# priyasundaresan/panda-lang-manip

Hardware: AMD Instinct MI355X
Metric: env steps/sec (batched) PandaPush-v3 at 1/2/4/8 MI355X vs PyBullet CPU (higher is better)
Workload: dtype f32; 1 GPU; PandaPush-v3 x65536/gpu; env_id=PandaPush-v3, task=push, control=ee, reward=sparse, batch_per_gpu=65536, global_batch=65536, substeps=20, parallelism=batch shard x1, lanes_per_env=1

## Files before the change

panda-lang-manip_amd/csrc/ps_scene.h:

```cpp
#pragma once

#include "ps_common.h"

namespace ps {

constexpr int SHAPE_BOX = PS_SHAPE_BOX;
constexpr int SHAPE_CYL = PS_SHAPE_CYLINDER;

struct Scene {
    V3 base;
    V3 half;
    float mass, mass2, fric;
    float table_cx, table_hx, table_hy;
    int has_table, has_plane;
};

struct Motors {
    float target[9], kp[9], kd[9], vel[9], imp[9];
};

struct Body {
    V3 pos;
    Q4 quat;
    V3 vel, omg;
// ... 77 lines not shown
PS_D V3 support_point(const Scene &sc) {
    if constexpr (SHAPE == SHAPE_CYL) {
        constexpr int order[PM_CYL_RIM_POINTS] = PM_CYL_RIM_ORDER;
        constexpr int cap = V / PM_CYL_RIM_POINTS;
        constexpr int j = order[V % PM_CYL_RIM_POINTS];
        constexpr float cs[8] = {1.0f, 0.70710678118654752f, 0.0f, -0.70710678118654752f,
                                 -1.0f, -0.70710678118654752f, 0.0f, 0.70710678118654752f};
        constexpr float sn[8] = {0.0f, 0.70710678118654752f, 1.0f, 0.70710678118654752f,
                                 0.0f, -0.70710678118654752f, -1.0f, -0.70710678118654752f};
        return mk(sc.half.x * cs[j], sc.half.x * sn[j], cap ? sc.half.z : -sc.half.z);
    } else {
        return mk((V & 1) ? sc.half.x : -sc.half.x, (V & 2) ? sc.half.y : -sc.half.y,
                  (V & 4) ? sc.half.z : -sc.half.z);
    }
}

template <int SHAPE>
PS_D float object_closest(const Scene &sc, V3 loc, V3 &cl, V3 &nl) {
    const V3 h = sc.half;
    if constexpr (SHAPE == SHAPE_CYL) {
        float r = h.x, hh = h.z;
        float rho = fast_sqrt(loc.x * loc.x + loc.y * loc.y);
        float zc = fminf(fmaxf(loc.z, -hh), hh);
        float irho = fast_rcp(rho);
        float s = rho > r ? r * irho : 1.0f;
        cl = mk(loc.x * s, loc.y * s, zc);
        V3 dif = loc - cl;
        float dn = fast_norm(dif);
        if (dn > 1e-9f) {
            nl = dif * fast_rcp(dn);
            return dn;
        }
        float side = r - rho, cap = hh - fabsf(loc.z);
        if (side < cap) {
            nl = rho > 1e-12f ? mk(loc.x * irho, loc.y * irho, 0.0f) : mk(1.0f, 0.0f, 0.0f);
            cl = mk(nl.x * r, nl.y * r, cl.z);
            return -side;
        }
        nl = mk(0.0f, 0.0f, loc.z >= 0.0f ? 1.0f : -1.0f);
        cl.z = nl.z * hh;
        return -cap;
    } else {
        cl = mk(fminf(fmaxf(loc.x, -h.x), h.x), fminf(fmaxf(loc.y, -h.y), h.y), fminf(fmaxf(loc.z, -h.z), h.z));
        V3 dif = loc - cl;
        float dn = norm(dif);
        if (dn > 1e-9f) {
            nl = dif * (1.0f / dn);
            return dn;
        }
        float bx = h.x - fabsf(loc.x), by = h.y - fabsf(loc.y), bz = h.z - fabsf(loc.z);
        int ax = 0;
        float best = bx;
        if (by < best) { best = by; ax = 1; }
        if (bz < best) { best = bz; ax = 2; }
        float sg;
        if (ax == 0) { sg = loc.x >= 0.0f ? 1.0f : -1.0f; nl = mk(sg, 0, 0); cl.x = sg * h.x; }
        else if (ax == 1) { sg = loc.y >= 0.0f ? 1.0f : -1.0f; nl = mk(0, sg, 0); cl.y = sg * h.y; }
        else { sg = loc.z >= 0.0f ? 1.0f : -1.0f; nl = mk(0, 0, sg); cl.z = sg * h.z; }
        return -best;
    }
}

PS_D void plane_space(V3 n, V3 &p, V3 &q) {
    if (fabsf(n.z) > 0.70710678118654752f) {
        float a = n.y * n.y + n.z * n.z, k = rsqrtf(a);
        p = mk(0.0f, -n.z * k, n.y * k);
        q = mk(a * k, -n.x * p.z, n.x * p.y);
    } else {
        float a = n.x * n.x + n.y * n.y, k = rsqrtf(a);
        p = mk(-n.y * k, n.x * k, 0.0f);
        q = mk(-n.z * p.y, n.z * p.x, a * k);
    }
}

constexpr int NG = PM_MAX_GROUND_CONTACTS;
constexpr int NR = PM_MAX_ROBOT_CONTACTS;
constexpr int NP = PM_MAX_PAIR_CONTACTS;
constexpr int LDS_STASH_OFFSET = NR * 27;
constexpr int LDS_STASH_FLOATS = 40;
constexpr int LDS_CACHE_OFFSET = LDS_STASH_OFFSET + LDS_STASH_FLOATS;
constexpr int LDS_CACHE_FLOATS = 10;
constexpr int LDS_FLOATS = LDS_CACHE_OFFSET + LDS_CACHE_FLOATS;
static_assert(LDS_FLOATS * 4 * 64 * 4 <= 160 * 1024, "four workgroups per CU");
constexpr int LDS_GND_OFFSET = NR * 27;
constexpr int LDS_GND_FLOATS = 6;
constexpr int LDS_FLOATS_STACK = LDS_GND_OFFSET + 2 * NG * LDS_GND_FLOATS;
static_assert(LDS_FLOATS_STACK * 4 * 64 * 4 <= 160 * 1024, "four Stack workgroups per CU");
constexpr int PAIR_FLOATS = 21;
constexpr int GSTASH_ROWS = LDS_STASH_FLOATS + 13 - 9;
constexpr int GSTASH_PAIR_OFFSET = GSTASH_ROWS;
constexpr int GSTASH_ZERO_FLOATS = 32;
constexpr int GRIP_MJ_SLOTS = NR;
constexpr int GSTASH_GRIP_OFFSET = GSTASH_PAIR_OFFSET + NP * PAIR_FLOATS;
constexpr int GRIP_FLOATS = GRIP_MJ_SLOTS * 9;
constexpr int GSTASH_FLOATS = GSTASH_GRIP_OFFSET + GRIP_FLOATS;
template <int NOBJ>
constexpr int lds_floats() {
    return NOBJ == 2 ? LDS_FLOATS_STACK : LDS_FLOATS;
}

struct GroundContact {
    V3 r;
    float rhs[3], lam[3], dinv[3];
    int id;
};

struct PairContact {
    V3 dir[3], rA, rB;
    float rhs[3], lam[3], dinv[3];
    bool a0;
};

struct RobotContact {
    float J[3][9];
    V3 dir[3];
    V3 rn[3];
    float rhs[3], lam[3], dinv[3], mu;
    bool o1;
};

typedef __attribute__((address_space(3))) float lds_float;
struct MJStore {
    lds_float *base;
    int stride;
    lds_float *cwo = nullptr;
    PS_D lds_float &at(int slot, int row, int k) const { return base[((slot * 3 + row) * 9 + k) * stride]; }
    PS_D lds_float &cache(int k) const { return base[(LDS_CACHE_OFFSET + k) * stride]; }
    PS_D lds_float &stash(int k) const { return base[(LDS_STASH_OFFSET + k) * stride]; }
    float *gst = nullptr;
    int64_t gst_stride = 0;
    uint32_t goff = 0;
    __attribute__((address_space(1))) float *gpair = nullptr;
    PS_D float &gstash(int k) const {
        float *row = gst + k * gst_stride;
        asm("" : "+s"(row));
        return *(float *)((char *)row + goff);
    }
    PS_D lds_float &gnd(int c, int k) const { return base[(LDS_GND_OFFSET + c * LDS_GND_FLOATS + k) * stride]; }
    PS_D float &pair(int c, int k) const { return *(float *)&gpair[c * PAIR_FLOATS + k]; }
    __attribute__((address_space(1))) float *ggrip = nullptr;
    PS_D float &grip(int c, int k) const { return *(float *)&ggrip[c * 9 + k]; }
    __attribute__((address_space(1))) float *gzero = nullptr;
    PS_D __attribute__((address_space(1))) float *pair_rows(int c, int n) const {
        return c < n ? gpair + c * PAIR_FLOATS : gzero;
    }
    PS_D __attribute__((address_space(1))) float *grip_rows(int c, int n) const {
        return c < n ? ggrip + c * 9 : gzero;
    }
    PS_D MJStore opaque() const {
        MJStore r = *this;
        asm volatile("" : "+v"(r.base));
        asm volatile("" : "+v"(r.goff));
        asm volatile("" : "+v"(r.gpair));
        asm volatile("" : "+v"(r.ggrip));
        return r;
    }
};

struct VelChange {
    f32x2 p[4];
    float z;
    PS_D float g(int a) const { return a == 8 ? z : p[a >> 1][a & 1]; }
    PS_D void s(int a, float v) {
        if (a == 8) z = v;
        else p[a >> 1][a & 1] = v;
    }
    PS_D f32x2 bc(int a) const {
        if (a == 8) return (f32x2){z, z};
        return (a & 1) ? __builtin_shufflevector(p[a >> 1], p[a >> 1], 1, 1)
                       : __builtin_shufflevector(p[a >> 1], p[a >> 1], 0, 0);
    }
    PS_D void apply(const float m[9], float sc) {
#pragma unroll
        for (int k = 0; k < 4; k++)
            p[k] = __builtin_elementwise_fma((f32x2){m[2 * k], m[2 * k + 1]}, (f32x2){sc, sc}, p[k]);
        z = fmaf(m[8], sc, z);
    }
    PS_D float dot(const float J[9]) const {
        float acc = 0.0f;
#pragma unroll
        for (int a = 0; a < 9; a++) acc = fmaf(J[a], g(a), acc);
        return acc;
    }
};

PS_D V3 pk_fma3(V3 a, float s, V3 c) {
    const f32x2 xy = __builtin_elementwise_fma((f32x2){a.x, a.y}, (f32x2){s, s}, (f32x2){c.x, c.y});
    return mk(xy.x, xy.y, fmaf(a.z, s, c.z));
}

PS_D float jrow_dot(const float J[9], const float v[9]) {
    float s = 0.0f;
#pragma unroll
    for (int d = 0; d < 9; d++) s += J[d] * v[d];
    return s;
}

struct Geo {
    V3 ax[9], org[7], bc[PM_NUM_BOXES], wc;
    M3 hR;
};

}
```

panda-lang-manip_amd/csrc/ps_substep.h:

```cpp
#pragma once

#include "ps_collide.h"
#include "ps_dynamics.h"
#include "ps_solver.h"
#include "ps_solver_group.h"

namespace ps {

#ifdef PS_PROFILE_PHASES
#define PS_COUNT_IT() prof_it++
#else
#define PS_COUNT_IT() do {} while (0)
#endif
#define PS_REGATE()                                                                        \
    do {                                                                                   \
        asm volatile("" : "+s"(gate_lim), "+s"(gate_pair), "+s"(gate_robot));              \
        for (int b_ = 0; b_ < NB; b_++) asm volatile("" : "+s"(gate_ground[b_]));         \
    } while (0)

struct LimitSide {
    float pen, sgn;
    bool on, combined;
    PS_D float split() const { return sgn * (-pen) * (float)PM_SPLIT_LIMIT_ERP; }
};
PS_D LimitSide limit_side(int d, int side, float qd_) {
    const double LO = dof_def(d).lo, HI = dof_def(d).hi;
    const float lo_h = (float)LO, lo_t = (float)(LO - (double)lo_h);
    const float hi_h = (float)HI, hi_t = (float)(HI - (double)hi_h);
    LimitSide s;
    s.pen = side ? (hi_h - qd_) + hi_t : (qd_ - lo_h) - lo_t;
    s.sgn = side ? -1.0f : 1.0f;
    s.on = s.pen <= 0.0f;
    s.combined = s.pen > (float)PM_SPLIT_PENETRATION_THRESHOLD;
    return s;
}

PS_D float split_of(int d, float qd_) {
    float split = 0.0f;
#pragma unroll
    for (int side = 0; side < 2; side++) {
        const LimitSide s = limit_side(d, side, qd_);
        if (s.on && !s.combined) split += s.split();
    }
    return split;
}

template <int NOBJ, int SHAPE, bool STD_MOTORS, int G = 1>
PS_D void substep(const Scene &sc, float q[9], float qd[9], const Motors &mt, Body *bd, const MJStore &lds,
                  const WarmCache<G, NOBJ> &wc PS_PROF_PARAM PS_DUMP_PARAM) {
    static_assert(NOBJ >= 0 && NOBJ <= 2, "objects");
    static_assert(NOBJ < 2 || SHAPE == SHAPE_BOX, "Stack stacks cubes");
    constexpr int NB = NOBJ > 0 ? NOBJ : 1;
    constexpr bool ANISO = SHAPE == SHAPE_CYL;
    const float dt = (float)PM_TIMESTEP;
    float Mi[45], hb[9];
    Geo geo;
    bias_forces(q, qd, hb);
    PS_PHASE(0);
    __builtin_amdgcn_sched_barrier(0);
    {
        Kin k;
        fk(q, k);
        static_for<0, 9>([&](auto D) {
            constexpr int d = decltype(D)::value;
            geo.ax[d] = dof_axis<d>(k);
            if constexpr (d < 7) geo.org[d] = k.f[d].o;
        });
        geo.hR = k.f[8].R;
        static_for<0, PM_NUM_BOXES>([&](auto BB) {
            constexpr int B = decltype(BB)::value;
            constexpr BoxDef b = box_def(B);
            geo.bc[B] = k.f[b.link].o + mul(k.f[b.link].R, mk((float)b.c[0], (float)b.c[1], (float)b.c[2])) + sc.base;
        });
        {
            constexpr SphereDef w = wrist_def();
            geo.wc = k.f[w.link].o + mul(k.f[w.link].R, mk((float)w.c[0], (float)w.c[1], (float)w.c[2])) + sc.base;
        }
        mass_matrix(k, Mi);
    }
#ifdef PS_PROFILE_PHASES
#pragma unroll
    for (int k = 0; k < 45; k++) asm volatile("" ::"v"(Mi[k]));
#endif
    PS_PHASE(1);
    __builtin_amdgcn_sched_barrier(0);
    spd_inverse(Mi);
#ifdef PS_PROFILE_PHASES
#pragma unroll
    for (int k = 0; k < 45; k++) asm volatile("" ::"v"(Mi[k]));
#endif
    PS_PHASE(2);
    __builtin_amdgcn_sched_barrier(0);
    int nr;
    {
        M3 oR[NB];
#pragma unroll
        for (int b = 0; b < NB; b++) oR[b] = NOBJ > 0 ? quat_to_mat(bd[b].quat) : M3{{1, 0, 0, 0, 1, 0, 0, 0, 1}};
        nr = robot_candidates<NOBJ, SHAPE, G>(sc, geo, bd, oR, lds PS_PROF_ARG);
    }
    PS_PHASE(17);
    __builtin_amdgcn_sched_barrier(0);
    float v1[9];
#pragma unroll
    for (int a = 0; a < 9; a++) {
        float s = 0.0f;
#pragma unroll
        for (int b = 0; b < 9; b++) s -= Mi[sidx(a, b)] * hb[b];
        v1[a] = qd[a] + dt * s;
    }
    V3 cw1[NB], cv1[NB];
    BodyDyn<SHAPE> od[NB];
#pragma unroll
    for (int b = 0; b < NB; b++) {
        cw1[b] = mk(0, 0, 0);
        cv1[b] = mk(0, 0, 0);
    }
#pragma unroll
    for (int b = 0; b < NOBJ; b++) {
        od[b] = body_dyn<SHAPE>(sc, bd[b], b == 0 ? sc.mass : sc.mass2);
        float cl = (float)PM_LINEAR_DAMPING + (float)PM_LINEAR_DAMPING * norm(bd[b].vel);
        float ca = (float)PM_ANGULAR_DAMPING + (float)PM_ANGULAR_DAMPING * norm(bd[b].omg);
        cv1[b] = bd[b].vel + (mk(0, 0, (float)PM_GRAVITY_Z) - bd[b].vel * cl) * dt;
        cw1[b] = bd[b].omg - bd[b].omg * (ca * dt);
        if constexpr (ANISO) {
            V3 I = local_inertia<SHAPE>(sc, b == 0 ? sc.mass : sc.mass2);
            S3 Iw = rotate_diag(od[b].R, I.x, I.y, I.z);
            V3 gyro = od[b].inv_inertia(cross(bd[b].omg, mul(Iw, bd[b].omg)));
            cw1[b] = cw1[b] - gyro * dt;
        }
    }

    float dinvj[9];
    float lim_rhs[9], lim_lam[9];
    unsigned lim_on = 0u, lim_up = 0u;
    float split_dq[9];
    float mot_rhs[9], mot_lam[9];
// ... 104 lines not shown
        float pl[NP];
        V3 ppt[NP];
        const int pn = (int)wc.load(PS_F_WPN);
#pragma unroll
        for (int k = 0; k < NP; k++) {
            pl[k] = wc.load(PS_F_WP + k);
            ppt[k] = mk(wc.load(PS_F_WPPT + 3 * k), wc.load(PS_F_WPPT + 3 * k + 1), wc.load(PS_F_WPPT + 3 * k + 2));
        }
#pragma unroll
        for (int c = 0; c < NP; c++) {
            PairContact &p = pc[c];
            if (c < np) {
                const PairCand &cd = cand[c];
                int A = cd.a0 ? 0 : 1;
                V3 dirs[3];
                dirs[0] = cd.n;
                plane_space(cd.n, dirs[1], dirs[2]);
                V3 rA = cd.pA - (A == 0 ? bd[0].pos : bd[1].pos), rB = cd.pB - (A == 0 ? bd[1].pos : bd[0].pos);
                p.a0 = cd.a0;
                p.rA = A == 0 ? rA : rB;
                p.rB = A == 0 ? rB : rA;
#pragma unroll
                for (int j = 0; j < 3; j++) {
                    V3 dj = dirs[j];
                    p.dir[j] = dj;
                    const V3 rnA = cross(rA, dj), rnB = cross(rB, dj);
                    float iIA = A == 0 ? od[0].iI : od[1].iI, iIB = A == 0 ? od[1].iI : od[0].iI;
                    float imA = A == 0 ? od[0].inv_m : od[1].inv_m, imB = A == 0 ? od[1].inv_m : od[0].inv_m;
                    float den = dot(rnA, rnA) * iIA + dot(rnB, rnB) * iIB + dot(dj, dj) * (imA + imB);
                    p.dinv[j] = safe_inv(den);
                    V3 wA = A == 0 ? cw1[0] : cw1[1], vA = A == 0 ? cv1[0] : cv1[1];
                    V3 wB = A == 0 ? cw1[1] : cw1[0], vB = A == 0 ? cv1[1] : cv1[0];
                    float rel = dot(rnA, wA) + dot(dj, vA) - dot(rnB, wB) - dot(dj, vB);
                    p.lam[j] = 0.0f;
                    p.rhs[j] = j == 0 ? normal_rhs(cd.dist, rel, p.dinv[0]) : -rel * p.dinv[j];
                }
                V3 lp = tmul(od[0].R, cd.pB - bd[0].pos);
                float best = (float)(PM_CONTACT_BREAKING_THRESHOLD * PM_CONTACT_BREAKING_THRESHOLD), l0 = 0.0f;
#pragma unroll
                for (int k = 0; k < NP; k++) {
                    V3 d = ppt[k] - lp;
                    float d2 = dot(d, d);
                    bool hit = k < pn && d2 < best;
                    best = hit ? d2 : best;
                    l0 = hit ? pl[k] : l0;
                }
                p.lam[0] = warm * l0;
                wc.store(PS_F_WPPT + 3 * c, lp.x);
                wc.store(PS_F_WPPT + 3 * c + 1, lp.y);
                wc.store(PS_F_WPPT + 3 * c + 2, lp.z);
            } else {
                p.a0 = true;
                p.rA = p.rB = mk(0, 0, 0);
#pragma unroll
                for (int j = 0; j < 3; j++) {
                    p.dir[j] = mk(0, 0, 0);
                    p.rhs[j] = p.lam[j] = p.dinv[j] = 0.0f;
                }
            }
            if (c < np) {
#pragma unroll
                for (int j = 0; j < 3; j++) {
                    lds.pair(c, 3 * j + 0) = p.dir[j].x; lds.pair(c, 3 * j + 1) = p.dir[j].y; lds.pair(c, 3 * j + 2) = p.dir[j].z;
                    lds.pair(c, 15 + j) = p.rhs[j];
                    lds.pair(c, 18 + j) = p.dinv[j];
                }
                lds.pair(c, 9) = p.rA.x; lds.pair(c, 10) = p.rA.y; lds.pair(c, 11) = p.rA.z;
                lds.pair(c, 12) = p.rB.x; lds.pair(c, 13) = p.rB.y; lds.pair(c, 14) = p.rB.z;
            }
        }
        wc.store(PS_F_WPN, (float)np);
    }
    RobotContact rc[NR];
    {
        PS_PHASE(18);
        float prl[NR];
#pragma unroll
        for (int k = 0; k < NR; k++) prl[k] = wc.load(PS_F_WR + k);
        const unsigned prid = (unsigned)wc.load(PS_F_WRID);
        unsigned nrid = 0u;
#pragma unroll
        for (int sl = 0; sl < NR; sl++) {
            RobotContact &c = rc[sl];
            if (sl < nr) {
                const RobotCand cd = RobotCand::load(lds, sl);
                V3 dirs[3];
                dirs[0] = cd.n;
                plane_space(cd.n, dirs[1], dirs[2]);
                c.mu = cd.mu;
                c.o1 = cd.obj == 1;
                bool on_obj = NOBJ > 0 && cd.obj >= 0;
                V3 p = cd.pA - sc.base;
                V3 opos = NOBJ == 2 && cd.obj == 1 ? bd[NB - 1].pos : bd[0].pos;
                V3 rB = cd.pB - opos;
                V3 ow = NOBJ == 2 && cd.obj == 1 ? cw1[NB - 1] : cw1[0];
                V3 ov = NOBJ == 2 && cd.obj == 1 ? cv1[NB - 1] : cv1[0];
                float oim = NOBJ == 2 && cd.obj == 1 ? od[NB - 1].inv_m : od[0].inv_m;
#pragma unroll
                for (int j = 0; j < 3; j++) {
                    V3 dj = dirs[j];
#pragma unroll
                    for (int D = 0; D < 7; D++) c.J[j][D] = dot(geo.ax[D], cross(p - geo.org[D], dj));
                    c.J[j][7] = cd.link == 9 ? dot(geo.ax[7], dj) : 0.0f;
                    c.J[j][8] = cd.link == 10 ? dot(geo.ax[8], dj) : 0.0f;
                    float den = 0.0f;
#pragma unroll
                    for (int a = 0; a < 9; a++) {
                        float s = 0.0f;
#pragma unroll
                        for (int b = 0; b < 9; b++) s += Mi[sidx(a, b)] * c.J[j][b];
                        lds.at(sl, j, a) = NOBJ == 2 ? c.J[j][a] : s;
                        if constexpr (NOBJ == 2)
                            if (j == 0) lds.grip(sl, a) = s;
                        den += c.J[j][a] * s;
                    }
                    float rel = jrow_dot(c.J[j], v1);
                    c.rn[j] = on_obj ? cross(rB, dj) : mk(0, 0, 0);
                    c.dir[j] = on_obj ? dj : mk(0, 0, 0);
                    if constexpr (NOBJ > 0) {
                        V3 w = ANISO ? od[0].inv_inertia(c.rn[j])
                                     : c.rn[j] * (NOBJ == 2 && cd.obj == 1 ? od[NB - 1].iI : od[0].iI);
                        if (on_obj) {
                            den += dot(c.rn[j], w) + dot(dj, dj) * oim;
                            rel -= dot(c.rn[j], ow) + dot(dj, ov);
                        }
                    }
                    c.dinv[j] = safe_inv(den);
                    c.lam[j] = 0.0f;
                    c.rhs[j] = j == 0 ? normal_rhs(cd.dist, rel, c.dinv[0]) : -rel * c.dinv[j];
                }
                c.lam[0] = warm * cache_lookup(prl, prid, (unsigned)cd.id);
                nrid |= (unsigned)cd.id << (5 * sl);
            } else {
                c.mu = 0.0f;
                c.o1 = false;
#pragma unroll
                for (int j = 0; j < 3; j++) {
#pragma unroll
                    for (int a = 0; a < 9; a++) {
                        c.J[j][a] = 0.0f;
                        lds.at(sl, j, a) = 0.0f;
                    }
                    c.dir[j] = c.rn[j] = mk(0, 0, 0);
                    c.rhs[j] = c.lam[j] = c.dinv[j] = 0.0f;
                }
            }
        }
        wc.store(PS_F_WRID, (float)nrid);
    }
    PS_PHASE(3);
    __builtin_amdgcn_sched_barrier(0);
    auto gk = [](int k) { return NOBJ == 2 && k >= 27 ? k - 9 : k; };
    auto put = [&](int k, float v) {
        if constexpr (NOBJ == 2) lds.gstash(gk(k)) = v;
        else lds.stash(k) = v;
    };
    auto get = [&](const MJStore &S, int k) -> float {
        if constexpr (NOBJ == 2) return S.gstash(gk(k));
        else return S.stash(k);
    };
#pragma unroll
    for (int d = 0; d < 9; d++) {
        put(d, q[d]);
        put(9 + d, v1[d]);
        if constexpr (NOBJ != 2) put(18 + d, split_dq[d]);
    }
    if constexpr (NOBJ > 0) {
        put(27, cw1[0].x); put(28, cw1[0].y); put(29, cw1[0].z);
        put(30, cv1[0].x); put(31, cv1[0].y); put(32, cv1[0].z);
        put(33, bd[0].pos.x); put(34, bd[0].pos.y); put(35, bd[0].pos.z);
        put(36, bd[0].quat.x); put(37, bd[0].quat.y); put(38, bd[0].quat.z); put(39, bd[0].quat.w);
    }
    if constexpr (NOBJ == 2) {
        put(40, cw1[1].x); put(41, cw1[1].y); put(42, cw1[1].z);
        put(43, cv1[1].x); put(44, cv1[1].y); put(45, cv1[1].z);
        put(46, bd[1].pos.x); put(47, bd[1].pos.y); put(48, bd[1].pos.z);
        put(49, bd[1].quat.x); put(50, bd[1].quat.y); put(51, bd[1].quat.z); put(52, bd[1].quat.w);
    }

    float dv[9];
#pragma unroll
    for (int d = 0; d < 9; d++) dv[d] = 0.0f;
    V3 dw[NB], dvl[NB];
#pragma unroll
    for (int b = 0; b < NB; b++) {
        dw[b] = mk(0, 0, 0);
        dvl[b] = mk(0, 0, 0);
    }
    float res;
    MJStore L = lds;

    auto wave_bits = [&](auto pred, int n) {
        unsigned m = 0u;
        for (int k = 0; k < n; k++) m |= __builtin_amdgcn_ballot_w64(pred(k)) ? 1u << k : 0u;
        return (unsigned)__builtin_amdgcn_readfirstlane((int)m);
    };
    unsigned gate_lim = wave_bits([&](int d) { return ((lim_on >> d) & 1u) != 0u; }, 9);
    unsigned gate_ground[NB];
#pragma unroll
    for (int b = 0; b < NB; b++) gate_ground[b] = wave_bits([&](int c) { return c < ng[b]; }, NG);
    unsigned gate_pair = wave_bits([&](int c) { return c < np; }, NP);
    unsigned gate_robot = wave_bits([&](int c) { return c < nr; }, NR);

#ifdef PS_PROFILE_PHASES
    int prof_it = 0;
#endif
    static_assert(PM_SOLVER_ITERATIONS % 2 == 0, "iteration pairs");
    if constexpr (G == 1) {
        VelChange dvv;
#pragma unroll
        for (int k = 0; k < 4; k++) dvv.p[k] = (f32x2){0.0f, 0.0f};
        dvv.z = 0.0f;
        auto mcol_apply = [&](int d, float f) {
            const int a0 = (d + 1) & ~1;
#pragma unroll
            for (int a = 0; a < 9; a++)
                if (a < a0 || a == 8) dvv.s(a, fmaf(Mi[sidx(a, d)], f, dvv.g(a)));
#pragma unroll
            for (int a = a0; a < 8; a += 2)
                dvv.p[a >> 1] = __builtin_elementwise_fma((f32x2){Mi[sidx(a, d)], Mi[sidx(a + 1, d)]}, (f32x2){f, f},
                                                          dvv.p[a >> 1]);
        };
        auto joint_row = [&](int d, float sgn, float rhs, float &lam, float lo, float hi) {
            float dl = rhs - dinvj[d] * (sgn * dvv.g(d));
            float nl = clamp_impulse(lam + dl, lo, hi);
            dl = nl - lam;
            lam = nl;
            mcol_apply(d, sgn * dl);
            res = res_max(res, joint_viol(dl, Mi[sidx(d, d)]));
        };
        auto limit_row = [&](int d) {
            if (PS_GATE(gate_lim & (1u << d), 0)) {
                float sgn = (lim_up >> d) & 1u ? -1.0f : 1.0f;
                float hi = (lim_on >> d) & 1u ? (float)PM_LIMIT_MAX_IMPULSE : 0.0f;
                joint_row(d, sgn, lim_rhs[d], lim_lam[d], 0.0f, hi);
            }
        };
        auto motor_row = [&](int d) {
            float imp = STD_MOTORS ? (float)(joint_force(d) * PM_TIMESTEP) : mt.imp[d];
            joint_row(d, 1.0f, mot_rhs[d], mot_lam[d], -imp, imp);
        };
        auto obj_add = [&](bool o1, V3 ddw, V3 ddv) {
            if constexpr (NOBJ == 2) {
                const float s1 = o1 ? 1.0f : 0.0f, s0 = o1 ? 0.0f : 1.0f;
                dw[0] = fma3(ddw, s0, dw[0]);
                dvl[0] = fma3(ddv, s0, dvl[0]);
                dw[NB - 1] = fma3(ddw, s1, dw[NB - 1]);
                dvl[NB - 1] = fma3(ddv, s1, dvl[NB - 1]);
            } else {
                dw[0] = dw[0] + ddw;
                dvl[0] = dvl[0] + ddv;
            }
        };
        auto obj_dw = [&](bool o1) { return NOBJ == 2 && o1 ? dw[NB - 1] : dw[0]; };
        auto obj_dv = [&](bool o1) { return NOBJ == 2 && o1 ? dvl[NB - 1] : dvl[0]; };
        auto pair_rel = [&](V3 rn0, V3 rn1, V3 d) {
            return dot(rn0, dw[0]) + dot(d, dvl[0]) - dot(rn1, dw[NB - 1]) - dot(d, dvl[NB - 1]);
        };
        auto pair_apply = [&](V3 rn0, V3 rn1, V3 d, float sdl) {
            dw[0] = pk_fma3(rn0, sdl * od[0].iI, dw[0]);
            dvl[0] = pk_fma3(d, sdl * od[0].inv_m, dvl[0]);
            dw[NB - 1] = pk_fma3(rn1, -sdl * od[NB - 1].iI, dw[NB - 1]);
            dvl[NB - 1] = pk_fma3(d, -sdl * od[NB - 1].inv_m, dvl[NB - 1]);
        };

        auto mi_apply = [&](const float g[9]) {
#pragma unroll
            for (int b = 0; b < 9; b++) mcol_apply(b, g[b]);
        };

        {
            MJStore W = lds.opaque();
#pragma unroll
            for (int b = 0; b < NOBJ; b++)
#pragma unroll
                for (int c = 0; c < NG; c++)
                    if (PS_GATE(gate_ground[b] & (1u << c), 1)) {
                        const float l0 = gc[b][c].lam[0];
                        V3 gr = gc[b][c].r;
                        if (NOBJ == 2) {
                            const int at = b * NG + c;
                            gr = mk(W.gnd(at, 0), W.gnd(at, 1), W.gnd(at, 2));
                        }
                        dw[b] = dw[b] + od[b].inv_inertia(mk(gr.y * l0, -gr.x * l0, 0.0f));
                        dvl[b].z = fmaf(l0, od[b].inv_m, dvl[b].z);
                    }
            if constexpr (NOBJ == 2) {
#pragma unroll
                for (int c = 0; c < NP; c++)
                    if (gate_pair & (1u << c)) {
                        const auto *pr = W.pair_rows(c, np);
                        auto pv = [&](int k) { return mk(pr[k], pr[k + 1], pr[k + 2]); };
                        const float sl = pc[c].a0 ? pc[c].lam[0] : -pc[c].lam[0];
                        const V3 d0 = pv(0);
                        pair_apply(cross(pv(9), d0), cross(pv(12), d0), d0, sl);
                    }
            }
#pragma unroll
            for (int c = 0; c < NR; c++)
                if (PS_GATE(gate_robot & (1u << c), c < 2)) {
                    const RobotContact &r = rc[c];
                    const float l0 = r.lam[0];
                    float Jl[9];
#pragma unroll
                    for (int a = 0; a < 9; a++) Jl[a] = NOBJ == 2 ? (float)W.at(c, 0, a) : r.J[0][a];
                    if constexpr (NOBJ == 2) {
                        float g[9];
#pragma unroll
                        for (int a = 0; a < 9; a++) g[a] = Jl[a] * l0;
                        mi_apply(g);
                    } else {
                        float w[9];
#pragma unroll
                        for (int a = 0; a < 9; a++) w[a] = W.at(c, 0, a);
#pragma unroll
                        for (int a = 0; a < 9; a++) dvv.s(a, fmaf(w[a], l0, dvv.g(a)));
                    }
                    if constexpr (NOBJ > 0) {
                        float im = NOBJ == 2 && r.o1 ? od[NB - 1].inv_m : od[0].inv_m;
                        V3 ddw = ANISO ? od[0].inv_inertia(r.rn[0] * -l0)
                                       : r.rn[0] * (-l0 * (NOBJ == 2 && r.o1 ? od[NB - 1].iI : od[0].iI));
                        obj_add(r.o1, ddw, r.dir[0] * (-l0 * im));
                    }
                }
        }

        float gmj[GRIP_MJ_SLOTS][9];
        auto object_normals = [&]() {
            if constexpr (NOBJ == 2) {
                float pf[NP][11];
                if constexpr (NOBJ == 2) {
                    if (gate_pair) {
#pragma unroll
                        for (int c = 0; c < NP; c++) {
                            const auto *pr = L.pair_rows(c, np);
#pragma unroll
                            for (int k = 0; k < 3; k++) {
                                pf[c][k] = pr[k];
                                pf[c][3 + k] = pr[9 + k];
                                pf[c][6 + k] = pr[12 + k];
                            }
                            pf[c][9] = pr[15];
                            pf[c][10] = pr[18];
                        }
                        __builtin_amdgcn_sched_barrier(0);
                    }
                    {
#pragma unroll
                        for (int c = 0; c < GRIP_MJ_SLOTS; c++)
                            if (gate_robot & (1u << c)) {
                                const auto *gr = L.grip_rows(c, nr);
#pragma unroll
                                for (int k = 0; k < 9; k++) gmj[c][k] = gr[k];
                            }
                        __builtin_amdgcn_sched_barrier(0);
                    }
                }
#pragma unroll
                for (int b = 0; b < NOBJ; b++) {
                    const float inv_m = od[b].inv_m;
#pragma unroll
                    for (int c = 0; c < NG; c++) {
                        GroundContact &g = gc[b][c];
                        V3 gr = g.r;
                        float grhs = g.rhs[0], gdinv = g.dinv[0];
                        if (NOBJ == 2) {
                            const int at = b * NG + c;
                            gr = mk(L.gnd(at, 0), L.gnd(at, 1), L.gnd(at, 2));
                            grhs = L.gnd(at, 3);
                            gdinv = c < ng[b] ? cube_ground_dinv(gr, 0, od[b].iI, inv_m) : 0.0f;
                        }
                        V3 rn = mk(gr.y, -gr.x, 0.0f);
                        float dl = grhs - gdinv * (rn.x * dw[b].x + rn.y * dw[b].y + dvl[b].z);
                        float nl = clamp_impulse(g.lam[0] + dl, 0.0f, (float)PM_CONTACT_UPPER);
                        dl = nl - g.lam[0];
                        g.lam[0] = nl;
                        if constexpr (ANISO) {
                            dw[b] = dw[b] + od[b].inv_inertia(mk(rn.x * dl, rn.y * dl, 0.0f));
                        } else {
                            float dI = dl * od[b].iI;
                            dw[b].x = fmaf(rn.x, dI, dw[b].x);
                            dw[b].y = fmaf(rn.y, dI, dw[b].y);
                        }
                        dvl[b].z = fmaf(dl, inv_m, dvl[b].z);
                        res = res_max(res, row_viol(dl, gdinv));
                    }
                }
                if constexpr (NOBJ == 2) {
                    if (gate_pair) {
#pragma unroll
                        for (int c = 0; c < NP; c++)
                            if (gate_pair & (1u << c)) {
                                PairContact &p = pc[c];
                                const float sg = p.a0 ? 1.0f : -1.0f;
                                const V3 d0 = mk(pf[c][0], pf[c][1], pf[c][2]);
                                const V3 rn0 = cross(mk(pf[c][3], pf[c][4], pf[c][5]), d0);
                                const V3 rn1 = cross(mk(pf[c][6], pf[c][7], pf[c][8]), d0);
                                float jv = sg * pair_rel(rn0, rn1, d0);
                                float dl = pf[c][9] - pf[c][10] * jv;
                                float nl = clamp_impulse(p.lam[0] + dl, 0.0f, (float)PM_CONTACT_UPPER);
                                dl = nl - p.lam[0];
                                p.lam[0] = nl;
                                pair_apply(rn0, rn1, d0, sg * dl);
                                res = res_max(res, row_viol(dl, pf[c][10]));
                            }
                    }
                }
            }
        };
        auto contacts = [&]() {
#pragma unroll
            for (int c = 0; c < NR; c++)
                if (PS_GATE(gate_robot & (1u << c), c < 2)) {
                    RobotContact &r = rc[c];
                    float mj[9], Jl[9];
#pragma unroll
                    for (int a = 0; a < 9; a++) Jl[a] = NOBJ == 2 ? (float)L.at(c, 0, a) : r.J[0][a];
                    if constexpr (NOBJ != 2) {
#pragma unroll
                        for (int a = 0; a < 9; a++) mj[a] = L.at(c, 0, a);
                    }
                    __builtin_amdgcn_sched_barrier(0);
                    float jv = dvv.dot(Jl);
                    if (NOBJ > 0) jv -= dot(r.rn[0], obj_dw(r.o1)) + dot(r.dir[0], obj_dv(r.o1));
                    float dl = r.rhs[0] - r.dinv[0] * jv;
                    float nl = clamp_impulse(r.lam[0] + dl, 0.0f, (float)PM_CONTACT_UPPER);
                    dl = nl - r.lam[0];
                    r.lam[0] = nl;
                    if constexpr (NOBJ == 2) {
                        dvv.apply(gmj[c], dl);
                    } else {
                        dvv.apply(mj, dl);
                    }
                    if constexpr (NOBJ == 1) {
                        dw[0] = ANISO ? dw[0] + od[0].inv_inertia_pk(r.rn[0] * -dl) : pk_fma3(r.rn[0], -dl * od[0].iI, dw[0]);
                        dvl[0] = pk_fma3(r.dir[0], -dl * od[0].inv_m, dvl[0]);
                    } else if constexpr (NOBJ == 2) {
                        float im = r.o1 ? od[NB - 1].inv_m : od[0].inv_m;
                        float iI = r.o1 ? od[NB - 1].iI : od[0].iI;
                        obj_add(r.o1, r.rn[0] * (-dl * iI), r.dir[0] * (-dl * im));
                    }
                    res = res_max(res, row_viol(dl, r.dinv[0]));
                }
            float pq[NP][16];
            if constexpr (NOBJ == 2) {
                if (gate_pair) {
#pragma unroll
                    for (int c = 0; c < NP; c++) {
                        const auto *pr = L.pair_rows(c, np);
#pragma unroll
                        for (int k = 0; k < 12; k++) pq[c][k] = pr[3 + k];
                        pq[c][12] = pr[16];
                        pq[c][13] = pr[17];
                        pq[c][14] = pr[19];
                        pq[c][15] = pr[20];
                    }
                    __builtin_amdgcn_sched_barrier(0);
                }
            }

#pragma unroll
            for (int b = 0; b < NOBJ; b++) {
                const float inv_m = od[b].inv_m;
#pragma unroll
                for (int c = 0; c < NG; c++)
                    if (PS_GATE(gate_ground[b] & (1u << c), 1)) {
                        GroundContact &g = gc[b][c];
                        V3 gr = g.r;
                        float grhs1 = g.rhs[1], grhs2 = g.rhs[2], gdinv1 = g.dinv[1], gdinv2 = g.dinv[2];
                        if (NOBJ == 2) {
                            const int at = b * NG + c;
                            gr = mk(L.gnd(at, 0), L.gnd(at, 1), L.gnd(at, 2));
                            grhs1 = L.gnd(at, 4);
                            grhs2 = L.gnd(at, 5);
                            const bool on = c < ng[b];
                            gdinv1 = on ? cube_ground_dinv(gr, 1, od[b].iI, inv_m) : 0.0f;
                            gdinv2 = on ? cube_ground_dinv(gr, 2, od[b].iI, inv_m) : 0.0f;
                        }
                        float dla, dlb;
                        {
#pragma clang fp contract(off)
                            const f32x2 gz = {gr.z, gr.z};
                            const f32x2 t = (f32x2){gr.x, gr.y} * (f32x2){dw[b].z, dw[b].z};
                            const f32x2 u = __builtin_elementwise_fma(gz, (f32x2){dw[b].x, dw[b].y}, -t);
                            const f32x2 w = u + (f32x2){-dvl[b].y, dvl[b].x};
                            const f32x2 lam12 = {g.lam[1], g.lam[2]};
                            const f32x2 s2 = lam12 + __builtin_elementwise_fma(-(f32x2){gdinv1, gdinv2}, w,
                                                                               (f32x2){grhs1, grhs2});
                            const float lim = gmu * g.lam[0];
                            const float m2 = NOBJ == 2 ? fmaf(s2.x, s2.x, s2.y * s2.y) : fmaf(s2.y, s2.y, s2.x * s2.x);
                            const float sc2 = cone_scale(m2, lim);
                            const f32x2 dl2 = __builtin_elementwise_fma(s2, (f32x2){sc2, sc2}, -lam12);
                            const f32x2 nl2 = s2 * (f32x2){sc2, sc2};
                            g.lam[1] = nl2.x;
                            g.lam[2] = nl2.y;
                            dla = dl2.x;
                            dlb = dl2.y;
                            if constexpr (ANISO) {
                                const f32x2 zab = gz * dl2;
                                dw[b] = dw[b] + od[b].inv_inertia_pk_unfused(mk(zab.x, zab.y, fmaf(-gr.x, dla, -gr.y * dlb)));
                            } else {
                                const f32x2 ab = dl2 * (f32x2){od[b].iI, od[b].iI};
                                const f32x2 wxy = __builtin_elementwise_fma(gz, ab, (f32x2){dw[b].x, dw[b].y});
                                dw[b].z = fmaf(-gr.y, ab.y, fmaf(-gr.x, ab.x, dw[b].z));
                                dw[b].x = wxy.x;
                                dw[b].y = wxy.y;
                            }
                            const f32x2 vxy = __builtin_elementwise_fma((f32x2){dlb, -dla}, (f32x2){inv_m, inv_m},
                                                                        (f32x2){dvl[b].x, dvl[b].y});
                            dvl[b].x = vxy.x;
                            dvl[b].y = vxy.y;
                        }
                        res = res_max(res, res_max(row_viol(dla, gdinv1), row_viol(dlb, gdinv2)));
                    }
            }
            if constexpr (NOBJ == 2) {
                const float pmu = sc.fric * sc.fric;
                if (gate_pair) {
#pragma unroll
                    for (int c = 0; c < NP; c++)
                        if (gate_pair & (1u << c)) {
                            PairContact &p = pc[c];
                            auto pv = [&](int k) { return mk(pq[c][k], pq[c][k + 1], pq[c][k + 2]); };
                            const float sg = p.a0 ? 1.0f : -1.0f;
                            const V3 d1 = pv(0), d2 = pv(3), r0 = pv(6), r1 = pv(9);
                            const V3 rn01 = cross(r0, d1), rn02 = cross(r0, d2), rn11 = cross(r1, d1), rn12 = cross(r1, d2);
                            float ja = sg * pair_rel(rn01, rn11, d1);
                            float jb = sg * pair_rel(rn02, rn12, d2);
                            float dla = pq[c][12] - pq[c][14] * ja, dlb = pq[c][13] - pq[c][15] * jb;
                            float sa = p.lam[1] + dla, sb = p.lam[2] + dlb;
                            float lim = pmu * p.lam[0];
                            float m2 = sa * sa + sb * sb;
                            float s = cone_scale(m2, lim);
                            sa *= s;
                            sb *= s;
                            dla = sa - p.lam[1];
                            dlb = sb - p.lam[2];
                            p.lam[1] = sa;
                            p.lam[2] = sb;
                            pair_apply(rn01, rn11, d1, sg * dla);
                            pair_apply(rn02, rn12, d2, sg * dlb);
                            res = res_max(res, res_max(row_viol(dla, pq[c][14]), row_viol(dlb, pq[c][15])));
                        }
                }
            }
#pragma unroll
            for (int c = 0; c < NR; c++)
                if (PS_GATE(gate_robot & (1u << c), c < 2)) {
                    RobotContact &r = rc[c];
                    float mj1[9], mj2[9], J1[9], J2[9];
#pragma unroll
                    for (int a = 0; a < 9; a++) {
                        J1[a] = NOBJ == 2 ? (float)L.at(c, 1, a) : r.J[1][a];
                        J2[a] = NOBJ == 2 ? (float)L.at(c, 2, a) : r.J[2][a];
                    }
                    if constexpr (NOBJ != 2) {
#pragma unroll
                        for (int a = 0; a < 9; a++) {
                            mj1[a] = L.at(c, 1, a);
                            mj2[a] = L.at(c, 2, a);
                        }
                    }
                    __builtin_amdgcn_sched_barrier(0);
                    float ja, jb;
                    if constexpr (NOBJ != 2) {
#pragma clang fp contract(off)
                        f32x2 j2 = {0.0f, 0.0f};
#pragma unroll
                        for (int a = 0; a < 9; a++) j2 = __builtin_elementwise_fma((f32x2){J1[a], J2[a]}, dvv.bc(a), j2);
                        ja = j2.x;
                        jb = j2.y;
                    } else {
                        ja = dvv.dot(J1);
                        jb = dvv.dot(J2);
                    }
                    if (NOBJ > 0) {
                        V3 ow = obj_dw(r.o1), ov = obj_dv(r.o1);
                        ja -= dot(r.rn[1], ow) + dot(r.dir[1], ov);
                        jb -= dot(r.rn[2], ow) + dot(r.dir[2], ov);
                    }
                    float dla, dlb;
                    if constexpr (NOBJ != 2) {
#pragma clang fp contract(off)
                        const f32x2 lam12 = {r.lam[1], r.lam[2]};
                        const f32x2 s2 = lam12 + __builtin_elementwise_fma(-(f32x2){r.dinv[1], r.dinv[2]}, (f32x2){ja, jb},
                                                                           (f32x2){r.rhs[1], r.rhs[2]});
                        const float lim = r.mu * r.lam[0];
                        const float sc2 = cone_scale(fmaf(s2.x, s2.x, s2.y * s2.y), lim);
                        const f32x2 dl2 = __builtin_elementwise_fma(s2, (f32x2){sc2, sc2}, -lam12);
                        const f32x2 nl2 = s2 * (f32x2){sc2, sc2};
                        r.lam[1] = nl2.x;
                        r.lam[2] = nl2.y;
                        dla = dl2.x;
                        dlb = dl2.y;
                    } else {
                        dla = r.rhs[1] - r.dinv[1] * ja;
                        dlb = r.rhs[2] - r.dinv[2] * jb;
                        float sa = r.lam[1] + dla, sb = r.lam[2] + dlb;
                        const float lim = r.mu * r.lam[0];
                        const float m2 = sa * sa + sb * sb;
                        const float s = cone_scale(m2, lim);
                        sa *= s;
                        sb *= s;
                        dla = sa - r.lam[1];
                        dlb = sb - r.lam[2];
                        r.lam[1] = sa;
                        r.lam[2] = sb;
                    }
                    if constexpr (NOBJ == 2) {
                        float g[9];
#pragma unroll
                        for (int a = 0; a < 9; a++) g[a] = fmaf(J2[a], dlb, J1[a] * dla);
                        mi_apply(g);
                    } else {
                        dvv.apply(mj1, dla);
                        dvv.apply(mj2, dlb);
                    }
                    if constexpr (NOBJ == 1) {
                        if constexpr (ANISO) {
                            dw[0] = dw[0] + od[0].inv_inertia_pk(fma3(r.rn[2], -dlb, r.rn[1] * -dla));
                        } else {
                            float aI = -dla * od[0].iI, bI = -dlb * od[0].iI;
                            dw[0] = pk_fma3(r.rn[2], bI, pk_fma3(r.rn[1], aI, dw[0]));
                        }
                        float am = -dla * od[0].inv_m, bm = -dlb * od[0].inv_m;
                        dvl[0] = pk_fma3(r.dir[2], bm, pk_fma3(r.dir[1], am, dvl[0]));
                    } else if constexpr (NOBJ == 2) {
                        float im = r.o1 ? od[NB - 1].inv_m : od[0].inv_m;
                        float iI = r.o1 ? od[NB - 1].iI : od[0].iI;
                        float aI = -dla * iI, bI = -dlb * iI;
                        V3 ddw = mk(fmaf(r.rn[2].x, bI, r.rn[1].x * aI), fmaf(r.rn[2].y, bI, r.rn[1].y * aI),
                                    fmaf(r.rn[2].z, bI, r.rn[1].z * aI));
                        float am = -dla * im, bm = -dlb * im;
                        V3 ddv = mk(fmaf(r.dir[2].x, bm, r.dir[1].x * am), fmaf(r.dir[2].y, bm, r.dir[1].y * am),
                                    fmaf(r.dir[2].z, bm, r.dir[1].z * am));
                        obj_add(r.o1, ddw, ddv);
                    }
                    res = res_max(res, res_max(row_viol(dla, r.dinv[1]), row_viol(dlb, r.dinv[2])));
                }
// ... 25 lines not shown
        for (int it = 0; it < PM_SOLVER_ITERATIONS; it += 2) {
            PS_COUNT_IT();
            L = lds.opaque();
            res = 0.0f;
            PS_REGATE();
            if constexpr (NOBJ == 1) {
#pragma unroll
                for (int k = 0; k < 45; k++) asm volatile("" : "+v"(Mi[k]));
            }
#pragma unroll
            for (int d = 8; d >= 0; d--) motor_row(d);
            ground_normals();
            object_normals();
            if (PS_GATE(gate_lim != 0u, 0)) {
#pragma unroll
                for (int d = 8; d >= 0; d--) limit_row(d);
            }
            contacts();
            if (res <= 0.0f) break;
            PS_COUNT_IT();
            L = lds.opaque();
            res = 0.0f;
            PS_REGATE();
            if (PS_GATE(gate_lim != 0u, 0)) {
#pragma unroll
                for (int d = 0; d < 9; d++) limit_row(d);
            }
#pragma unroll
            for (int d = 0; d < 9; d++) motor_row(d);
            ground_normals();
            object_normals();
            contacts();
            if (res <= 0.0f) break;
        }
#pragma unroll
        for (int a = 0; a < 9; a++) dv[a] = dvv.g(a);
    } else {
        group_pgs<NOBJ, SHAPE, STD_MOTORS, G>(mt, Mi, lds, gate_lim, lim_up, lim_on, gate_ground[0], gate_robot,
                                              dinvj, lim_rhs, lim_lam, mot_rhs, mot_lam, gc[0], rc, od[0], gmu,
                                              dv, dw[0], dvl[0] PS_PROF_COUNT_ARG PS_DUMP_ARG);
    }

#pragma unroll
    for (int b = 0; b < NOBJ; b++)
#pragma unroll
        for (int c = 0; c < NG; c++) wc.store((b == 0 ? PS_F_WG0 : PS_F_WG1) + c, gc[b][c].lam[0]);
    if constexpr (NOBJ == 2) {
#pragma unroll
        for (int c = 0; c < NP; c++) wc.store(PS_F_WP + c, pc[c].lam[0]);
    }
#pragma unroll
    for (int c = 0; c < NR; c++) wc.store(PS_F_WR + c, rc[c].lam[0]);

    PS_PHASE(4);
#ifdef PS_PROFILE_PHASES
    {
        int wmax = prof_it, wnr = nr;
#pragma unroll
        for (int o = 32; o >= 1; o >>= 1) {
            wmax = max(wmax, __shfl_xor(wmax, o));
            wnr = max(wnr, __shfl_xor(wnr, o));
        }
        pt.acc[8] += prof_it;
        pt.acc[9] += wmax;
#pragma unroll
        for (int k = PS_ITP_WORDS - 1; k > 0; k--) pt.itp[k] = (pt.itp[k] << 16) | (pt.itp[k - 1] >> 16);
        pt.itp[0] = (pt.itp[0] << 16) | (uint32_t)min(prof_it, 255) | ((uint32_t)nr << 8) | ((uint32_t)np << 11);
        pt.acc[10] += 1;
        pt.acc[11] += wnr;
        unsigned ngnd = 0;
        for (int b = 0; b < NB; b++) ngnd += __builtin_popcount(gate_ground[b]);
        pt.acc[12] += __builtin_popcount(gate_pair);
        pt.acc[13] += ngnd;
        pt.acc[14] += __builtin_popcount(gate_robot);
        pt.acc[15] += gate_lim != 0u;
    }
#endif
    {
        MJStore S = lds.opaque();
#pragma unroll
        for (int d = 0; d < 9; d++) {
            q[d] = get(S, d);
            v1[d] = get(S, 9 + d);
            split_dq[d] = NOBJ == 2 ? split_of(d, q[d]) : get(S, 18 + d);
        }
        if constexpr (NOBJ > 0) {
            cw1[0] = mk(get(S, 27), get(S, 28), get(S, 29));
            cv1[0] = mk(get(S, 30), get(S, 31), get(S, 32));
            bd[0].pos = mk(get(S, 33), get(S, 34), get(S, 35));
            bd[0].quat = Q4{get(S, 36), get(S, 37), get(S, 38), get(S, 39)};
        }
        if constexpr (NOBJ == 2) {
            cw1[1] = mk(get(S, 40), get(S, 41), get(S, 42));
            cv1[1] = mk(get(S, 43), get(S, 44), get(S, 45));
            bd[1].pos = mk(get(S, 46), get(S, 47), get(S, 48));
            bd[1].quat = Q4{get(S, 49), get(S, 50), get(S, 51), get(S, 52)};
        }
    }
#pragma unroll
    for (int d = 0; d < 9; d++) {
        qd[d] = v1[d] + dv[d];
        q[d] += dt * qd[d] + split_dq[d];
    }
#pragma unroll
    for (int b = 0; b < NOBJ; b++) {
        Body &cb = bd[b];
        cb.omg = cw1[b] + dw[b];
        cb.vel = cv1[b] + dvl[b];
        cb.pos = cb.pos + cb.vel * dt;
        float ang = norm(cb.omg);
        if (ang * dt > 0.5f * 1.5707963267948966f) ang = 0.5f * 1.5707963267948966f / dt;
        float f = ang < 0.001f ? (0.5f * dt - (dt * dt * dt) * 0.020833333333f * ang * ang) : sinf(0.5f * ang * dt) / ang;
        Q4 dq = Q4{cb.omg.x * f, cb.omg.y * f, cb.omg.z * f, cosf(0.5f * ang * dt)};
        Q4 nq = qmul(dq, cb.quat);
        float nn = rsqrtf(nq.x * nq.x + nq.y * nq.y + nq.z * nq.z + nq.w * nq.w);
        cb.quat = Q4{nq.x * nn, nq.y * nn, nq.z * nn, nq.w * nn};
    }
    PS_PHASE(5);
}

#undef PS_COUNT_IT
#undef PS_REGATE

}
```

Baseline: 24.28 million env-steps/s.

## Pack robot-contact M^-1 J rows into lane-contiguous float4 LDS chunks

For single-object, single-lane configurations, the per-contact M^-1 J rows are now stored in LDS as 16-byte chunks contiguous per lane, so the solver reads and writes them with vector LDS operations instead of nine strided scalar accesses per row. The stash moves to a smaller region, and the limit split term is recomputed at the end instead of being stored. Inactive contact slots are zeroed with vector stores. The trade-off is extra recompute of the split term and a different LDS bank-access pattern, which may introduce bank conflicts with the 3-float lane offset.

```diff
diff --git a/panda-lang-manip_amd/csrc/ps_scene.h b/panda-lang-manip_amd/csrc/ps_scene.h
--- a/panda-lang-manip_amd/csrc/ps_scene.h
+++ b/panda-lang-manip_amd/csrc/ps_scene.h
@@ -183,6 +183,15 @@
 constexpr int LDS_CACHE_FLOATS = 10;
 constexpr int LDS_FLOATS = LDS_CACHE_OFFSET + LDS_CACHE_FLOATS;
 static_assert(LDS_FLOATS * 4 * 64 * 4 <= 160 * 1024, "four workgroups per CU");
+constexpr int LDS_CHUNK_FLOATS = 28;
+constexpr int LDS_CHUNKS = LDS_CHUNK_FLOATS / 4;
+constexpr int LDS1_STASH_OFFSET = NR * LDS_CHUNK_FLOATS;
+constexpr int LDS1_STASH_FLOATS = LDS_STASH_FLOATS - 9;
+static_assert(LDS1_STASH_OFFSET + LDS1_STASH_FLOATS <= LDS_CACHE_OFFSET, "the one-lane stash below the contact cache");
+template <int NOBJ, int G>
+constexpr bool chunked_lds() {
+    return G == 1 && NOBJ <= 1;
+}
 constexpr int LDS_GND_OFFSET = NR * 27;
 constexpr int LDS_GND_FLOATS = 6;
 constexpr int LDS_FLOATS_STACK = LDS_GND_OFFSET + 2 * NG * LDS_GND_FLOATS;
@@ -221,6 +230,8 @@
 };
 
 typedef __attribute__((address_space(3))) float lds_float;
+typedef float f32x4 __attribute__((ext_vector_type(4)));
+typedef __attribute__((address_space(3))) f32x4 lds_f32x4;
 struct MJStore {
     lds_float *base;
     int stride;
@@ -228,6 +239,25 @@
     PS_D lds_float &at(int slot, int row, int k) const { return base[((slot * 3 + row) * 9 + k) * stride]; }
     PS_D lds_float &cache(int k) const { return base[(LDS_CACHE_OFFSET + k) * stride]; }
     PS_D lds_float &stash(int k) const { return base[(LDS_STASH_OFFSET + k) * stride]; }
+    PS_D lds_f32x4 &chunk(int slot, int c) const {
+        return ((lds_f32x4 *)(base + 3 * (int)threadIdx.x))[(slot * LDS_CHUNKS + c) * 64];
+    }
+    PS_D void chunk_row(int slot, int, float m[9]) const {
+        const f32x4 a = chunk(slot, 0), b = chunk(slot, 1), z = chunk(slot, 6);
+        m[0] = a.x; m[1] = a.y; m[2] = a.z; m[3] = a.w;
+        m[4] = b.x; m[5] = b.y; m[6] = b.z; m[7] = b.w;
+        m[8] = z.x;
+    }
+    PS_D void chunk_rows12(int slot, float m1[9], float m2[9]) const {
+        const f32x4 a = chunk(slot, 2), b = chunk(slot, 3), c = chunk(slot, 4), d = chunk(slot, 5), z = chunk(slot, 6);
+        m1[0] = a.x; m1[1] = a.y; m1[2] = a.z; m1[3] = a.w;
+        m1[4] = b.x; m1[5] = b.y; m1[6] = b.z; m1[7] = b.w;
+        m2[0] = c.x; m2[1] = c.y; m2[2] = c.z; m2[3] = c.w;
+        m2[4] = d.x; m2[5] = d.y; m2[6] = d.z; m2[7] = d.w;
+        m1[8] = z.y;
+        m2[8] = z.z;
+    }
+    PS_D lds_float &stash1(int k) const { return base[(LDS1_STASH_OFFSET + k) * stride]; }
     float *gst = nullptr;
     int64_t gst_stride = 0;
     uint32_t goff = 0;
diff --git a/panda-lang-manip_amd/csrc/ps_substep.h b/panda-lang-manip_amd/csrc/ps_substep.h
--- a/panda-lang-manip_amd/csrc/ps_substep.h
+++ b/panda-lang-manip_amd/csrc/ps_substep.h
@@ -52,6 +52,7 @@
     static_assert(NOBJ < 2 || SHAPE == SHAPE_BOX, "Stack stacks cubes");
     constexpr int NB = NOBJ > 0 ? NOBJ : 1;
     constexpr bool ANISO = SHAPE == SHAPE_CYL;
+    constexpr bool CHUNKED = chunked_lds<NOBJ, G>();
     const float dt = (float)PM_TIMESTEP;
     float Mi[45], hb[9];
     Geo geo;
@@ -322,8 +323,14 @@
 #pragma unroll
         for (int sl = 0; sl < NR; sl++) {
             RobotContact &c = rc[sl];
+            RobotCand cd0{};
+            if constexpr (CHUNKED) {
+                cd0 = RobotCand::load(lds, sl);
+                __builtin_amdgcn_wave_barrier();
+            }
+            float mjc[LDS_CHUNK_FLOATS] = {};
             if (sl < nr) {
-                const RobotCand cd = RobotCand::load(lds, sl);
+                const RobotCand cd = CHUNKED ? cd0 : RobotCand::load(lds, sl);
                 V3 dirs[3];
                 dirs[0] = cd.n;
                 plane_space(cd.n, dirs[1], dirs[2]);
@@ -349,10 +356,15 @@
                         float s = 0.0f;
 #pragma unroll
                         for (int b = 0; b < 9; b++) s += Mi[sidx(a, b)] * c.J[j][b];
-                        lds.at(sl, j, a) = NOBJ == 2 ? c.J[j][a] : s;
+                        if constexpr (CHUNKED) mjc[a < 8 ? 8 * j + a : 24 + j] = s;
+                        else lds.at(sl, j, a) = NOBJ == 2 ? c.J[j][a] : s;
                         if constexpr (NOBJ == 2)
                             if (j == 0) lds.grip(sl, a) = s;
                         den += c.J[j][a] * s;
+                    }
+                    if constexpr (CHUNKED) {
+                        lds.chunk(sl, 2 * j) = (f32x4){mjc[8 * j], mjc[8 * j + 1], mjc[8 * j + 2], mjc[8 * j + 3]};
+                        lds.chunk(sl, 2 * j + 1) = (f32x4){mjc[8 * j + 4], mjc[8 * j + 5], mjc[8 * j + 6], mjc[8 * j + 7]};
                     }
                     float rel = jrow_dot(c.J[j], v1);
                     c.rn[j] = on_obj ? cross(rB, dj) : mk(0, 0, 0);
@@ -369,6 +381,7 @@
                     c.lam[j] = 0.0f;
                     c.rhs[j] = j == 0 ? normal_rhs(cd.dist, rel, c.dinv[0]) : -rel * c.dinv[j];
                 }
+                if constexpr (CHUNKED) lds.chunk(sl, 6) = (f32x4){mjc[24], mjc[25], mjc[26], 0.0f};
                 c.lam[0] = warm * cache_lookup(prl, prid, (unsigned)cd.id);
                 nrid |= (unsigned)cd.id << (5 * sl);
             } else {
@@ -379,31 +392,39 @@
 #pragma unroll
                     for (int a = 0; a < 9; a++) {
                         c.J[j][a] = 0.0f;
-                        lds.at(sl, j, a) = 0.0f;
+                        if constexpr (!CHUNKED)
+                            lds.at(sl, j, a) = 0.0f;
                     }
                     c.dir[j] = c.rn[j] = mk(0, 0, 0);
                     c.rhs[j] = c.lam[j] = c.dinv[j] = 0.0f;
                 }
+                if constexpr (CHUNKED) {
+#pragma unroll
+                    for (int k = 0; k < LDS_CHUNKS; k++) lds.chunk(sl, k) = (f32x4){0.0f, 0.0f, 0.0f, 0.0f};
+                }
             }
         }
         wc.store(PS_F_WRID, (float)nrid);
     }
     PS_PHASE(3);
     __builtin_amdgcn_sched_barrier(0);
-    auto gk = [](int k) { return NOBJ == 2 && k >= 27 ? k - 9 : k; };
+    constexpr bool SPLIT_REBUILT = NOBJ == 2 || CHUNKED;
+    auto gk = [](int k) { return SPLIT_REBUILT && k >= 27 ? k - 9 : k; };
     auto put = [&](int k, float v) {
         if constexpr (NOBJ == 2) lds.gstash(gk(k)) = v;
+        else if constexpr (CHUNKED) lds.stash1(gk(k)) = v;
         else lds.stash(k) = v;
     };
     auto get = [&](const MJStore &S, int k) -> float {
         if constexpr (NOBJ == 2) return S.gstash(gk(k));
+        else if constexpr (CHUNKED) return S.stash1(gk(k));
         else return S.stash(k);
     };
 #pragma unroll
     for (int d = 0; d < 9; d++) {
         put(d, q[d]);
         put(9 + d, v1[d]);
-        if constexpr (NOBJ != 2) put(18 + d, split_dq[d]);
+        if constexpr (!SPLIT_REBUILT) put(18 + d, split_dq[d]);
     }
     if constexpr (NOBJ > 0) {
         put(27, cw1[0].x); put(28, cw1[0].y); put(29, cw1[0].z);
@@ -551,8 +572,11 @@
                         mi_apply(g);
                     } else {
                         float w[9];
-#pragma unroll
-                        for (int a = 0; a < 9; a++) w[a] = W.at(c, 0, a);
+                        if constexpr (CHUNKED) W.chunk_row(c, 0, w);
+                        else {
+#pragma unroll
+                            for (int a = 0; a < 9; a++) w[a] = W.at(c, 0, a);
+                        }
 #pragma unroll
                         for (int a = 0; a < 9; a++) dvv.s(a, fmaf(w[a], l0, dvv.g(a)));
                     }
@@ -656,7 +680,9 @@
                     float mj[9], Jl[9];
 #pragma unroll
                     for (int a = 0; a < 9; a++) Jl[a] = NOBJ == 2 ? (float)L.at(c, 0, a) : r.J[0][a];
-                    if constexpr (NOBJ != 2) {
+                    if constexpr (CHUNKED) {
+                        L.chunk_row(c, 0, mj);
+                    } else if constexpr (NOBJ != 2) {
 #pragma unroll
                         for (int a = 0; a < 9; a++) mj[a] = L.at(c, 0, a);
                     }
@@ -794,7 +820,9 @@
                         J1[a] = NOBJ == 2 ? (float)L.at(c, 1, a) : r.J[1][a];
                         J2[a] = NOBJ == 2 ? (float)L.at(c, 2, a) : r.J[2][a];
                     }
-                    if constexpr (NOBJ != 2) {
+                    if constexpr (CHUNKED) {
+                        L.chunk_rows12(c, mj1, mj2);
+                    } else if constexpr (NOBJ != 2) {
 #pragma unroll
                         for (int a = 0; a < 9; a++) {
                             mj1[a] = L.at(c, 1, a);
@@ -986,7 +1014,7 @@
         for (int d = 0; d < 9; d++) {
             q[d] = get(S, d);
             v1[d] = get(S, 9 + d);
-            split_dq[d] = NOBJ == 2 ? split_of(d, q[d]) : get(S, 18 + d);
+            split_dq[d] = SPLIT_REBUILT ? split_of(d, q[d]) : get(S, 18 + d);
         }
         if constexpr (NOBJ > 0) {
             cw1[0] = mk(get(S, 27), get(S, 28), get(S, 29));
```

New measurement: 25.23 million env-steps/s, median of 6. 1.04x the previous value.
